# VisionDepth/VisionDepth3D

Measured on AMD Instinct MI355X. Metric: stereo-pairs/sec end-to-end (depth+warp+fill+mux), higher is better.
Workload: dtype f32; 1 GPU; 4k-dav2b-dibr; frame=3840x2160, format=Half-SBS, depth_model=depth-anything-v2-base, depth_net_dtype=float32 (the reference's precision), pixel_overlap=True, pixel_streams=2, clip_frames_all_ranks=32, params=render_cli.py defaults + dof_strength 2.0, dense DOF order (parity mode)

## Files before the change

visiondepth3d_amd/csrc/vd3d_attn.hip:

```cpp
#include "vd3d_dev.h"
#include "vd3d_kernels.h"

#include <mutex>

typedef short at_bf8 __attribute__((ext_vector_type(8)));
typedef float at_f16 __attribute__((ext_vector_type(16)));
typedef uint32_t at_u4 __attribute__((ext_vector_type(4)));

#define AT_D 64
#define AT_BQ 256
#define AT_BK 64
#define AT_NT 512
#define AT_NTERM(MODE) ((MODE) == 0 ? 3 : 2)
#define AT_TILE(MODE) (4 * AT_NTERM(MODE) * 2 * 64 * 16)
#define AT_STAGE(MODE) (2 * AT_TILE(MODE))
#define AT_NSTAGE 3
#define AT_LDS(MODE) (AT_NSTAGE * AT_STAGE(MODE))
#define AT_QBLK(MODE) (4 * AT_NTERM(MODE) * 2 * 32)
#define AT_QKV_SCALE 16.0f
#define AT_P_SCALE 1024.0f
#define AT_OP 272

struct vd_at_args {
  int B, H, T;
// ... 130 lines not shown
    uint8_t* dst = at_lds + buf * STAGE + op * TILE + pp * (AT_NT * 16) + wave_base;
    __builtin_amdgcn_global_load_lds((at_glb_vp)src, (at_lds_vp)dst, 16, 0, 0);
  };

  at_f16 oacc[2];
#pragma unroll
  for (int dm = 0; dm < 2; ++dm)
#pragma unroll
    for (int r = 0; r < 16; ++r) oacc[dm][r] = 0.f;
  float m_run = -INFINITY, l_half = 0.f;

  const int last_tile = a.nkv - 1;
  auto tile_c = [&](int t) { return t < last_tile ? t : last_tile; };
#pragma unroll
  for (int p = 0; p < 6; ++p) dma(0, 0, p);
#pragma unroll
  for (int p = 0; p < 3; ++p) dma(tile_c(1), 1, p);
#pragma unroll
  for (int p = 3; p < 6; ++p) dma(tile_c(1), 1, p);
#pragma unroll
  for (int p = 0; p < 3; ++p) dma(tile_c(2), 2, p);
  if (NP == 3) asm volatile("s_waitcnt vmcnt(6)" ::: "memory"); else asm volatile("s_waitcnt vmcnt(4)" ::: "memory");
  __builtin_amdgcn_s_barrier();

  const int frag_off = (kh * 64 + li) * 16;
  auto st_step = [&](const uint8_t* sk, int ks, at_f16 (&sa)[2]) {
    at_bf8 kf[2][NTERM];
#pragma unroll
    for (int m = 0; m < 2; ++m)
#pragma unroll
      for (int t = 0; t < NTERM; ++t) kf[m][t] = *reinterpret_cast<const at_bf8*>(sk + frag_off + ((ks * NTERM + t) * 2) * 1024 + m * 512);
    AT_MM6(sa[0], kf[0], sa[1], kf[1], qf[ks])
  };
#define AT_CHUNK_HINT(n)                                           \
  __builtin_amdgcn_sched_group_barrier(0x100, 6, 0);               \
  _Pragma("unroll") for (int i_ = 0; i_ < 12; ++i_) {              \
    __builtin_amdgcn_sched_group_barrier(0x008, 1, 0);             \
    __builtin_amdgcn_sched_group_barrier(0x002, n, 0);             \
  }                                                                \
  __builtin_amdgcn_sched_barrier(0);

  at_f16 sacc[2];
#pragma unroll
  for (int m = 0; m < 2; ++m)
#pragma unroll
    for (int r = 0; r < 16; ++r) sacc[m][r] = 0.f;
#pragma unroll
  for (int ks = 0; ks < 4; ++ks) st_step(at_lds, ks, sacc);
  asm volatile("s_waitcnt lgkmcnt(0)" ::: "memory");
  __builtin_amdgcn_s_barrier();

  int cur = 0;
  for (int it = 0; it < a.nkv; ++it) {
    const int s1 = cur == 2 ? 0 : cur + 1, s2 = cur >= 1 ? cur - 1 : 2;
    const uint8_t* sk1 = at_lds + s1 * STAGE;
    const uint8_t* sv = at_lds + cur * STAGE + TILE;
    float z[2][16];
#pragma unroll
    for (int m = 0; m < 2; ++m)
#pragma unroll
      for (int r = 0; r < 16; ++r) z[m][r] = sacc[m][r] * a.c;
    if ((it + 1) * AT_BK > a.T) {
#pragma unroll
      for (int m = 0; m < 2; ++m)
#pragma unroll
        for (int r = 0; r < 16; ++r)
          if (it * AT_BK + 32 * m + (r & 3) + 8 * (r >> 2) + 4 * kh >= a.T) z[m][r] = -INFINITY;
    }
    at_f16 sn[2];
#pragma unroll
    for (int m = 0; m < 2; ++m)
#pragma unroll
      for (int r = 0; r < 16; ++r) sn[m][r] = 0.f;
    dma(tile_c(it + 3), cur, 0);
    __builtin_amdgcn_sched_barrier(0);
    st_step(sk1, 0, sn);
    float mx = -INFINITY;
#pragma unroll
    for (int m = 0; m < 2; ++m)
#pragma unroll
      for (int r = 0; r < 16; ++r) mx = fmaxf(mx, z[m][r]);
    mx = fmaxf(mx, __shfl_xor(mx, 32, 64));
    const float m_new = fmaxf(m_run, mx);
    const float alpha = __builtin_amdgcn_exp2f(m_run - m_new);
    m_run = m_new;
    AT_CHUNK_HINT(2)
    float ps = 0.f;
#pragma unroll
    for (int m = 0; m < 2; ++m) {
      dma(tile_c(it + 3), cur, 1 + m);
      __builtin_amdgcn_sched_barrier(0);
      st_step(sk1, 1 + m, sn);
#pragma unroll
      for (int r = 0; r < 16; ++r) { z[m][r] = __builtin_amdgcn_exp2f(z[m][r] - m_new); ps += z[m][r]; }
      AT_CHUNK_HINT(4)
    }
    dma(tile_c(it + 2), s2, 3);
    __builtin_amdgcn_sched_barrier(0);
    st_step(sk1, 3, sn);
    l_half = l_half * alpha + ps;
#pragma unroll
    for (int dm = 0; dm < 2; ++dm)
#pragma unroll
      for (int r = 0; r < 16; ++r) oacc[dm][r] *= alpha;
    at_bf8 pf[2][NTERM];
    at_split8_m<MODE>(&z[0][0], AT_P_SCALE, pf[0]);
    AT_CHUNK_HINT(7)
#pragma unroll
    for (int ks = 0; ks < 4; ++ks) {
      if (ks < 2) { dma(tile_c(it + 2), s2, 4 + ks); __builtin_amdgcn_sched_barrier(0); }
      if (ks < 3) at_split8_m<MODE>(&z[(ks + 1) >> 1][8 * ((ks + 1) & 1)], AT_P_SCALE, pf[(ks + 1) & 1]);
      at_bf8 vf[2][NTERM];
#pragma unroll
      for (int dm = 0; dm < 2; ++dm)
#pragma unroll
        for (int t = 0; t < NTERM; ++t) vf[dm][t] = *reinterpret_cast<const at_bf8*>(sv + frag_off + ((ks * NTERM + t) * 2) * 1024 + dm * 512);
      AT_MM6(oacc[0], vf[0], oacc[1], vf[1], pf[ks & 1])
      AT_CHUNK_HINT(4)
    }
    if (NP == 3) asm volatile("s_waitcnt vmcnt(6) lgkmcnt(0)" ::: "memory"); else asm volatile("s_waitcnt vmcnt(4) lgkmcnt(0)" ::: "memory");
    __builtin_amdgcn_s_barrier();
#pragma unroll
    for (int m = 0; m < 2; ++m) sacc[m] = sn[m];
    cur = s1;
  }
#undef AT_CHUNK_HINT
  asm volatile("s_waitcnt vmcnt(0)" ::: "memory");
  __builtin_amdgcn_s_barrier();

  const float l_tot = l_half + __shfl_xor(l_half, 32, 64);
  const float inv = MODE == 1 ? 1.0f / (l_tot * (AT_P_SCALE * AT_QKV_SCALE)) : 1.0f / l_tot;
  uint8_t* ow = at_lds + wave * (32 * AT_OP);
#pragma unroll
  for (int dm = 0; dm < 2; ++dm)
#pragma unroll
    for (int g = 0; g < 4; ++g) {
      const float4 v4 = {oacc[dm][4 * g] * inv, oacc[dm][4 * g + 1] * inv, oacc[dm][4 * g + 2] * inv, oacc[dm][4 * g + 3] * inv};
      *reinterpret_cast<float4*>(ow + li * AT_OP + (32 * dm + 8 * g + 4 * kh) * 4) = v4;
    }
  asm volatile("s_waitcnt lgkmcnt(0)" ::: "memory");
  const int b = bh / a.H, h = bh - b * a.H;
#pragma unroll
  for (int i = 0; i < 8; ++i) {
    const int row = i * 4 + (lane >> 4), c4 = lane & 15;
    const int q = q0 + row;
    const float4 v4 = *reinterpret_cast<const float4*>(ow + row * AT_OP + c4 * 16);
    if (q < a.T) *reinterpret_cast<float4*>(out + (((size_t)b * a.T + q) * a.H + h) * AT_D + c4 * 4) = v4;
  }
}

#define AF_TILE (AT_BK * AT_D * 4)
#define AF_STAGE (2 * AF_TILE)
#define AF_LDS (AT_NSTAGE * AF_STAGE)
VD_DEV void af_st(const uint8_t* __restrict__ sk, const float (&qf)[32], int li, int kh, at_f16 (&s)[2]) {
  const int kswz = (li & 15) << 4;
#pragma unroll
  for (int m = 0; m < 2; ++m)
#pragma unroll
    for (int r = 0; r < 16; ++r) s[m][r] = 0.f;
#pragma unroll
  for (int g = 0; g < 8; ++g) {
    float4 kf[2];
#pragma unroll
    for (int m = 0; m < 2; ++m) kf[m] = *reinterpret_cast<const float4*>(sk + (32 * m + li) * 256 + (((8 * kh + g) << 4) ^ kswz));
#pragma unroll
    for (int m = 0; m < 2; ++m) s[m] = __builtin_amdgcn_mfma_f32_32x32x2f32(kf[m].x, qf[4 * g], s[m], 0, 0, 0);
#pragma unroll
    for (int m = 0; m < 2; ++m) s[m] = __builtin_amdgcn_mfma_f32_32x32x2f32(kf[m].y, qf[4 * g + 1], s[m], 0, 0, 0);
#pragma unroll
    for (int m = 0; m < 2; ++m) s[m] = __builtin_amdgcn_mfma_f32_32x32x2f32(kf[m].z, qf[4 * g + 2], s[m], 0, 0, 0);
#pragma unroll
    for (int m = 0; m < 2; ++m) s[m] = __builtin_amdgcn_mfma_f32_32x32x2f32(kf[m].w, qf[4 * g + 3], s[m], 0, 0, 0);
  }
}
VD_DEV void af_pv(const uint8_t* __restrict__ sv, const at_f16 (&p)[2], int li, int kh, at_f16 (&oacc)[2]) {
#pragma unroll
  for (int m = 0; m < 2; ++m)
#pragma unroll
    for (int r = 0; r < 16; ++r) {
      const float2 vv = *reinterpret_cast<const float2*>(sv + (32 * m + (r & 3) + 8 * (r >> 2) + 4 * kh) * 256 + li * 8);
      oacc[0] = __builtin_amdgcn_mfma_f32_32x32x2f32(vv.x, p[m][r], oacc[0], 0, 0, 0);
      oacc[1] = __builtin_amdgcn_mfma_f32_32x32x2f32(vv.y, p[m][r], oacc[1], 0, 0, 0);
    }
}

__global__ __launch_bounds__(AT_NT) void k_attn_f32(const float* __restrict__ qkv, float* __restrict__ out, vd_at_args a) {
  extern __shared__ __attribute__((aligned(16))) uint8_t at_lds[];
  int bh, qb;
  {
    const int wg = blockIdx.x, x = wg & 7, idx = wg >> 3;
    const int g = idx / a.nqb;
    qb = idx - g * a.nqb;
    bh = g * 8 + x;
    if (bh >= a.B * a.H) return;
  }
  const int tid = threadIdx.x, lane = tid & 63, wave = __builtin_amdgcn_readfirstlane(tid >> 6);
  const int li = lane & 31, kh = lane >> 5;
  const int q0 = qb * AT_BQ + wave * 32;
  const int b = bh / a.H, h = bh - b * a.H;
  const size_t tok_stride = (size_t)3 * a.H * AT_D;
  const float* base = qkv + (size_t)b * a.T * tok_stride + h * AT_D;

  const int drow = tid >> 4, dpos = tid & 15, kchunk = dpos ^ (drow & 15);
  auto dma = [&](int tile, int stage) {
    uint8_t* dst = at_lds + stage * AF_STAGE + wave * 1024;
#pragma unroll
    for (int p = 0; p < 2; ++p) {
      const int tok = min(tile * AT_BK + drow + 32 * p, a.T - 1);
      const float* src = base + (size_t)tok * tok_stride + a.H * AT_D;
      __builtin_amdgcn_global_load_lds((at_glb_vp)(src + kchunk * 4), (at_lds_vp)(dst + p * 8192), 16, 0, 0);
      __builtin_amdgcn_global_load_lds((at_glb_vp)(src + a.H * AT_D + dpos * 4), (at_lds_vp)(dst + AF_TILE + p * 8192), 16, 0, 0);
    }
  };

  float qf[32];
  {
    const float4* qp = reinterpret_cast<const float4*>(base + (size_t)min(q0 + li, a.T - 1) * tok_stride + 32 * kh);
#pragma unroll
    for (int g = 0; g < 8; ++g) {
      const float4 v = qp[g];
      qf[4 * g] = v.x * a.c; qf[4 * g + 1] = v.y * a.c; qf[4 * g + 2] = v.z * a.c; qf[4 * g + 3] = v.w * a.c;
    }
  }
  dma(0, 0);
  if (a.nkv > 1) {
    dma(1, 1);
    asm volatile("s_waitcnt vmcnt(4)" ::: "memory");
  } else {
    asm volatile("s_waitcnt vmcnt(0)" ::: "memory");
  }
  __builtin_amdgcn_s_barrier();

  at_f16 oacc[2];
#pragma unroll
  for (int dm = 0; dm < 2; ++dm)
#pragma unroll
    for (int r = 0; r < 16; ++r) oacc[dm][r] = 0.f;
  float m_run = -INFINITY, l_half = 0.f;
  int cur = 0;
  for (int it = 0; it < a.nkv; ++it) {
    const bool ahead = it + 2 < a.nkv;
    if (ahead) dma(it + 2, cur == 0 ? 2 : cur - 1);
    const uint8_t* sk = at_lds + cur * AF_STAGE;
    const uint8_t* sv = sk + AF_TILE;
    at_f16 s[2];
    af_st(sk, qf, li, kh, s);
    if ((it + 1) * AT_BK > a.T) {
#pragma unroll
      for (int m = 0; m < 2; ++m)
#pragma unroll
        for (int r = 0; r < 16; ++r)
          if (it * AT_BK + 32 * m + (r & 3) + 8 * (r >> 2) + 4 * kh >= a.T) s[m][r] = -INFINITY;
    }
    float mx = s[0][0];
#pragma unroll
    for (int m = 0; m < 2; ++m)
#pragma unroll
      for (int r = 0; r < 16; ++r) mx = fmaxf(mx, s[m][r]);
    mx = fmaxf(mx, __shfl_xor(mx, 32, 64));
    const float m_new = fmaxf(m_run, mx);
    if (__any(m_new > m_run)) {
      const float alpha = __builtin_amdgcn_exp2f(m_run - m_new);
#pragma unroll
      for (int dm = 0; dm < 2; ++dm)
#pragma unroll
        for (int r = 0; r < 16; ++r) oacc[dm][r] *= alpha;
      l_half *= alpha;
      m_run = m_new;
    }
    float ps = 0.f;
#pragma unroll
    for (int m = 0; m < 2; ++m)
#pragma unroll
      for (int r = 0; r < 16; ++r) { s[m][r] = __builtin_amdgcn_exp2f(s[m][r] - m_run); ps += s[m][r]; }
    l_half += ps;
    af_pv(sv, s, li, kh, oacc);
    if (ahead) asm volatile("s_waitcnt vmcnt(4) lgkmcnt(0)" ::: "memory"); else asm volatile("s_waitcnt vmcnt(0) lgkmcnt(0)" ::: "memory");
    __builtin_amdgcn_s_barrier();
    cur = cur == 2 ? 0 : cur + 1;
  }

  const float l_tot = l_half + __shfl_xor(l_half, 32, 64);
  const int q = q0 + li;
  if (q < a.T) {
    float* op = out + (((size_t)b * a.T + q) * a.H + h) * AT_D + 8 * kh;
#pragma unroll
    for (int g = 0; g < 4; ++g) {
      const float4 lo = {oacc[0][4 * g] / l_tot, oacc[1][4 * g] / l_tot, oacc[0][4 * g + 1] / l_tot, oacc[1][4 * g + 1] / l_tot};
      const float4 hi = {oacc[0][4 * g + 2] / l_tot, oacc[1][4 * g + 2] / l_tot, oacc[0][4 * g + 3] / l_tot, oacc[1][4 * g + 3] / l_tot};
      *reinterpret_cast<float4*>(op + 16 * g) = lo;
      *reinterpret_cast<float4*>(op + 16 * g + 4) = hi;
    }
  }
}

static bool at_lds_optin(const void* fn, int lds, bool (&done)[64]) {
  static std::mutex mu;
  int dev = 0;
  if (hipGetDevice(&dev) != hipSuccess || dev < 0 || dev >= 64) return false;
  std::lock_guard<std::mutex> lock(mu);
  if (!done[dev]) {
    if (hipFuncSetAttribute(fn, hipFuncAttributeMaxDynamicSharedMemorySize, lds) != hipSuccess) return false;
    done[dev] = true;
  }
  return true;
}

bool vd_launch_attn_f32(hipStream_t s, const float* qkv, int B, int T, int H, int D, float scale, float* out) {
  if (B < 1 || T < 1 || H < 1 || D != AT_D || (long long)B * H > 65535) return false;
  if ((reinterpret_cast<uintptr_t>(qkv) & 15) || (reinterpret_cast<uintptr_t>(out) & 15)) return false;
  static bool attr_set[64] = {};
  if (!at_lds_optin(reinterpret_cast<const void*>(k_attn_f32), AF_LDS, attr_set)) return false;
  vd_at_args a;
  a.B = B; a.H = H; a.T = T;
  a.nq32 = (T + 31) / 32; a.nkv = (T + AT_BK - 1) / AT_BK; a.nqb = (T + AT_BQ - 1) / AT_BQ;
  a.c = scale * 1.44269504088896340736f;
  const int groups = (B * H + 7) / 8;
  hipLaunchKernelGGL(k_attn_f32, dim3((unsigned)(8 * groups * a.nqb)), dim3(AT_NT), AF_LDS, s, qkv, out, a);
  return true;
}

static bool at_mode_ok(int mode) { return mode == 0 || mode == 1; }
long long vd_attn_x3_workspace_bytes(int B, int T, int H, int D, int mode) {
  if (B < 1 || T < 1 || H < 1 || D != AT_D || !at_mode_ok(mode)) return -1;
  const long long nq32 = (T + 31) / 32, nkv = (T + AT_BK - 1) / AT_BK;
  const long long qblk = mode == 0 ? AT_QBLK(0) : AT_QBLK(1), tile = mode == 0 ? AT_TILE(0) : AT_TILE(1);
  return (long long)B * H * (nq32 * qblk * 16 + 2 * nkv * tile);
}

template <int MODE>
static bool at_launch(hipStream_t s, const float* qkv, int B, int T, int H, float scale, void* ws, float* out) {
  static bool attr_set[64] = {};
  if (!at_lds_optin(reinterpret_cast<const void*>(k_attn_bf16x3<MODE>), AT_LDS(MODE), attr_set)) return false;
  vd_at_args a;
  a.B = B; a.H = H; a.T = T;
  a.nq32 = (T + 31) / 32; a.nkv = (T + AT_BK - 1) / AT_BK; a.nqb = (T + AT_BQ - 1) / AT_BQ;
  a.c = scale * 1.44269504088896340736f;
  if (MODE == 1) a.c *= 1.0f / (AT_QKV_SCALE * AT_QKV_SCALE);
  uint4* Qimg = reinterpret_cast<uint4*>(ws);
  uint4* Kimg = Qimg + (size_t)B * H * a.nq32 * AT_QBLK(MODE);
  uint4* Vimg = Kimg + (size_t)B * H * a.nkv * (AT_TILE(MODE) / 16);
  const int rows_max = a.nkv * 64 > a.nq32 * 32 ? a.nkv * 64 : a.nq32 * 32;
  hipLaunchKernelGGL(k_attn_x3_prep<MODE>, dim3((unsigned)((rows_max * 8 + 255) / 256), (unsigned)(B * H), 3), dim3(256), 0, s, qkv, a, Qimg, Kimg, Vimg);
  const int groups = (B * H + 7) / 8;
  hipLaunchKernelGGL(k_attn_bf16x3<MODE>, dim3((unsigned)(8 * groups * a.nqb)), dim3(AT_NT), AT_LDS(MODE), s, Qimg, Kimg, Vimg, out, a);
  return true;
}

bool vd_launch_attn_x3(hipStream_t s, const float* qkv, int B, int T, int H, int D, float scale, void* ws, float* out, int mode) {
  if (vd_attn_x3_workspace_bytes(B, T, H, D, mode) < 0) return false;
  if ((reinterpret_cast<uintptr_t>(qkv) & 15) || (reinterpret_cast<uintptr_t>(ws) & 15) || (reinterpret_cast<uintptr_t>(out) & 15)) return false;
  if ((long long)B * H > 65535) return false;
  return mode == 0 ? at_launch<0>(s, qkv, B, T, H, scale, ws, out) : at_launch<1>(s, qkv, B, T, H, scale, ws, out);
}
```

visiondepth3d_amd/csrc/vd3d_depthprep.hip:

```cpp
#include "vd3d_dev.h"
#include "vd3d_kernels.h"

#define DP_TX 32
#define DP_TY 8
#define DP_KMAX 24

struct vd_prep_args {
  int B, H, W, th, tw;
  float scale_h, scale_w;
  float mean[3], stdv[3];
  int in_rows_max, in_cols_max;
};

VD_DEV float dp_cubic(float x) {
  const float a = -0.5f;
  x = fabsf(x);
  if (x < 1.f) return ((a + 2.f) * x - (a + 3.f)) * x * x + 1.f;
  if (x < 2.f) return (((x - 5.f) * x + 8.f) * x - 4.f) * a;
  return 0.f;
}
VD_DEV int dp_weights(int i, int in, float scale, float* w, int* first) {
  const float support = scale >= 1.f ? 2.f * scale : 2.f;
  const float invscale = scale >= 1.f ? 1.f / scale : 1.f;
  const float center = scale * ((float)i + 0.5f);
  int xmin = (int)(center - support + 0.5f); xmin = xmin < 0 ? 0 : xmin;
  int xend = (int)(center + support + 0.5f); xend = xend > in ? in : xend;
  int n = xend - xmin; n = n > DP_KMAX ? DP_KMAX : n;
  float total = 0.f;
  for (int j = 0; j < n; ++j) { const float v = dp_cubic(((float)(j + xmin) - center + 0.5f) * invscale); w[j] = v; total += v; }
  for (int j = 0; j < n; ++j) w[j] = total != 0.f ? w[j] / total : w[j];
  *first = xmin;
  return n;
}
VD_DEV uint16_t dp_bf16(float f) {
  const uint32_t b = __float_as_uint(f);
  return (uint16_t)((b + 0x7fffu + ((b >> 16) & 1u)) >> 16);
}

VD_DEV void dp_store(uint16_t* o, float f) { *o = dp_bf16(f); }
VD_DEV void dp_store(float* o, float f) { *o = f; }

template <typename OT>
__global__ __launch_bounds__(256) void k_depth_prep(const uint8_t* __restrict__ frames, vd_prep_args a, OT* __restrict__ out) {
  extern __shared__ unsigned char smem[];
  float* wx = reinterpret_cast<float*>(smem);
  float* wy = wx + DP_TX * DP_KMAX;
  int* x0s = reinterpret_cast<int*>(wy + DP_TY * DP_KMAX);
  int* y0s = x0s + 2 * DP_TX;
  float* hb = reinterpret_cast<float*>(y0s + 2 * DP_TY);
  uint8_t* tile = reinterpret_cast<uint8_t*>(hb + (size_t)a.in_rows_max * DP_TX * 3);
  const int tid = threadIdx.x;
  const int ox0 = blockIdx.x * DP_TX, oy0 = blockIdx.y * DP_TY, b = blockIdx.z;
  if (tid < DP_TX) {
    int f = 0, n = 0;
    if (ox0 + tid < a.tw) n = dp_weights(ox0 + tid, a.W, a.scale_w, wx + tid * DP_KMAX, &f);
    x0s[tid] = f; x0s[DP_TX + tid] = n;
  } else if (tid >= 64 && tid < 64 + DP_TY) {
    const int t = tid - 64;
    int f = 0, n = 0;
    if (oy0 + t < a.th) n = dp_weights(oy0 + t, a.H, a.scale_h, wy + t * DP_KMAX, &f);
    y0s[t] = f; y0s[DP_TY + t] = n;
  }
  __syncthreads();
  const int nx = min(DP_TX, a.tw - ox0), ny = min(DP_TY, a.th - oy0);
  const int c_lo = x0s[0], c_hi = x0s[nx - 1] + x0s[DP_TX + nx - 1];
  const int r_lo = y0s[0], r_hi = y0s[ny - 1] + y0s[DP_TY + ny - 1];
  const int ncol = min(c_hi - c_lo, a.in_cols_max), nrow = min(r_hi - r_lo, a.in_rows_max);
  const uint8_t* src = frames + (size_t)b * a.H * a.W * 3;
  const int rowbytes = ncol * 3;
  for (int t = tid; t < nrow * rowbytes; t += 256) {
    const int r = t / rowbytes, cb = t - r * rowbytes;
    tile[(size_t)r * a.in_cols_max * 3 + cb] = src[((size_t)(r_lo + r) * a.W + c_lo) * 3 + cb];
  }
  __syncthreads();
  for (int t = tid; t < nrow * DP_TX; t += 256) {
    const int r = t / DP_TX, ox = t - r * DP_TX;
    float s0 = 0.f, s1 = 0.f, s2 = 0.f;
    if (ox < nx) {
      const int n = x0s[DP_TX + ox];
      const uint8_t* p = tile + (size_t)r * a.in_cols_max * 3 + (size_t)(x0s[ox] - c_lo) * 3;
      const float* w = wx + ox * DP_KMAX;
      for (int j = 0; j < n; ++j) {
        const float wj = w[j];
        s0 += (float)p[3 * j + 2] * wj; s1 += (float)p[3 * j + 1] * wj; s2 += (float)p[3 * j] * wj;
      }
    }
    float* h = hb + ((size_t)r * DP_TX + ox) * 3;
    h[0] = s0; h[1] = s1; h[2] = s2;
  }
  __syncthreads();
  const int ox = tid & (DP_TX - 1), oy = tid / DP_TX;
  if (ox < nx && oy < ny) {
    const int n = y0s[DP_TY + oy], rb = y0s[oy] - r_lo;
    const float* w = wy + oy * DP_KMAX;
    float s[3] = {0.f, 0.f, 0.f};
    for (int j = 0; j < n; ++j) {
      const float* h = hb + ((size_t)(rb + j) * DP_TX + ox) * 3;
      const float wj = w[j];
      s[0] += h[0] * wj; s[1] += h[1] * wj; s[2] += h[2] * wj;
    }
    OT* o = out + (((size_t)b * a.th + (oy0 + oy)) * a.tw + (ox0 + ox)) * 3;
#pragma unroll
    for (int c = 0; c < 3; ++c) dp_store(o + c, ((s[c] / 255.0f) - a.mean[c]) / a.stdv[c]);
  }
}

bool vd_launch_depth_prep(hipStream_t s, const uint8_t* frames, int B, int H, int W, int th, int tw, const float mean[3],
                          const float stdv[3], int dtype, void* out_nhwc) {
  if (dtype != VD3D_DT_BF16 && dtype != VD3D_DT_F32) return false;
  vd_prep_args a;
  a.B = B; a.H = H; a.W = W; a.th = th; a.tw = tw;
  a.scale_h = (float)H / (float)th; a.scale_w = (float)W / (float)tw;
  const float sup_w = a.scale_w >= 1.f ? 2.f * a.scale_w : 2.f, sup_h = a.scale_h >= 1.f ? 2.f * a.scale_h : 2.f;
  if ((int)(2.f * sup_w) + 2 > DP_KMAX || (int)(2.f * sup_h) + 2 > DP_KMAX) return false;
  for (int c = 0; c < 3; ++c) { a.mean[c] = mean[c]; a.stdv[c] = stdv[c]; }
  a.in_cols_max = (int)(a.scale_w * DP_TX + 2.f * sup_w) + 4;
  a.in_rows_max = (int)(a.scale_h * DP_TY + 2.f * sup_h) + 4;
  size_t lds = sizeof(float) * (DP_TX + DP_TY) * DP_KMAX + sizeof(int) * 2 * (DP_TX + DP_TY) +
               sizeof(float) * (size_t)a.in_rows_max * DP_TX * 3 + (size_t)a.in_rows_max * a.in_cols_max * 3;
  lds = (lds + 15) & ~(size_t)15;
  if (lds > 150 * 1024) return false;
  static bool attr[64] = {false};
  int dev = 0;
  (void)hipGetDevice(&dev);
  if (dev >= 0 && dev < 64 && !attr[dev]) {
    (void)hipFuncSetAttribute((const void*)k_depth_prep<uint16_t>, hipFuncAttributeMaxDynamicSharedMemorySize, 160 * 1024);
    (void)hipFuncSetAttribute((const void*)k_depth_prep<float>, hipFuncAttributeMaxDynamicSharedMemorySize, 160 * 1024);
    attr[dev] = true;
  }
  dim3 g((tw + DP_TX - 1) / DP_TX, (th + DP_TY - 1) / DP_TY, B);
  if (dtype == VD3D_DT_F32) hipLaunchKernelGGL(k_depth_prep<float>, g, dim3(256), lds, s, frames, a, reinterpret_cast<float*>(out_nhwc));
  else hipLaunchKernelGGL(k_depth_prep<uint16_t>, g, dim3(256), lds, s, frames, a, reinterpret_cast<uint16_t*>(out_nhwc));
  return true;
}
```

visiondepth3d_amd/csrc/vd3d_handoff.hip:

```cpp
#include "vd3d_dev.h"
#include "vd3d_kernels.h"

struct vd_handoff_args { int B, ph, pw, H, W, invert, same; float sh, sw; };

VD_DEV float cubic1(float x, float A) { return ((A + 2.f) * x - (A + 3.f)) * x * x + 1.f; }
VD_DEV float cubic2(float x, float A) { return ((A * x - 5.f * A) * x + 8.f * A) * x - 4.f * A; }
VD_DEV void cubic_coeffs(float t, float c[4]) {
  const float A = -0.75f;
  c[0] = cubic2(t + 1.f, A); c[1] = cubic1(t, A); c[2] = cubic1(1.f - t, A); c[3] = cubic2((1.f - t) + 1.f, A);
}
VD_DEV float bicubic_at(const float* __restrict__ p, const vd_handoff_args& a, const float cy[4], int iy, int x) {
  const float rx = vd_fma(a.sw, (float)x + 0.5f, -0.5f);
  const float fx = floorf(rx);
  const int ix = (int)fx;
  float cx[4];
  cubic_coeffs(rx - fx, cx);
  int xs[4];
#pragma unroll
  for (int j = 0; j < 4; ++j) { int xx = ix - 1 + j; xs[j] = xx < 0 ? 0 : (xx > a.pw - 1 ? a.pw - 1 : xx); }
  float acc = 0.f;
#pragma unroll
  for (int i = 0; i < 4; ++i) {
    int yy = iy - 1 + i; yy = yy < 0 ? 0 : (yy > a.ph - 1 ? a.ph - 1 : yy);
    const float* row = p + (size_t)yy * a.pw;
    float r = 0.f;
#pragma unroll
    for (int j = 0; j < 4; ++j) r += row[xs[j]] * cx[j];
    acc += r * cy[i];
  }
  return acc;
}
VD_DEV uint32_t f2key(float v) { uint32_t b = __float_as_uint(v); return (b & 0x80000000u) ? ~b : (b | 0x80000000u); }
VD_DEV float key2f(uint32_t k) { uint32_t b = (k & 0x80000000u) ? (k & 0x7fffffffu) : ~k; return __uint_as_float(b); }

__global__ void k_handoff_init(uint32_t* mm, int B) {
  int i = blockIdx.x * blockDim.x + threadIdx.x;
  if (i < B) { mm[3 * i] = 0xffffffffu; mm[3 * i + 1] = 0u; mm[3 * i + 2] = 0u; }
}

#define HO_ROWS 32
template <bool WRITE>
__global__ __launch_bounds__(256) void k_handoff(const float* __restrict__ pred, vd_handoff_args a, uint32_t* __restrict__ mm,
                                                 uint8_t* __restrict__ out) {
  const int b = blockIdx.z;
  const float* p = pred + (size_t)b * a.ph * a.pw;
  const int xq = (blockIdx.x * 64 + (threadIdx.x & 63)) * 4;
  float bmn = INFINITY, bmx = -INFINITY;
  int bbad = 0;
  for (int ry_ = 0; ry_ < HO_ROWS / 4; ++ry_) {
  const int y = blockIdx.y * HO_ROWS + ry_ * 4 + (threadIdx.x >> 6);
  float v[4] = {0.f, 0.f, 0.f, 0.f};
  const bool row_ok = y < a.H;
  if (row_ok && xq < a.W) {
    if (a.same) {
#pragma unroll
      for (int q = 0; q < 4; ++q) if (xq + q < a.W) v[q] = p[(size_t)y * a.W + xq + q];
    } else {
      const float ry = vd_fma(a.sh, (float)y + 0.5f, -0.5f);
      const float fy = floorf(ry);
      float cy[4];
      cubic_coeffs(ry - fy, cy);
#pragma unroll
      for (int q = 0; q < 4; ++q) if (xq + q < a.W) v[q] = bicubic_at(p, a, cy, (int)fy, xq + q);
    }
  }
  if (!WRITE) {
    float mn = INFINITY, mx = -INFINITY;
    int bad = 0;
    if (row_ok)
#pragma unroll
      for (int q = 0; q < 4; ++q)
        if (xq + q < a.W) { bad |= (v[q] != v[q]); mn = v[q] < mn ? v[q] : mn; mx = v[q] > mx ? v[q] : mx; }
    bmn = fminf(bmn, mn); bmx = fmaxf(bmx, mx); bbad |= bad;
  } else {
    if (!row_ok || xq >= a.W) continue;
    const float mn = key2f(mm[3 * b]), mx = key2f(mm[3 * b + 1]);
    const bool flat = mm[3 * b + 2] != 0u || (mx - mn) < (float)1e-6;
    const float den = (mx - mn) + (float)1e-6;
    uint32_t pack = 0;
#pragma unroll
    for (int q = 0; q < 4; ++q) {
      uint8_t u = 0;
      if (!flat) {
        float n = ((v[q] - mn) / den) * 255.f;
        n = n < 0.f ? 0.f : (n > 255.f ? 255.f : n);
        u = (uint8_t)n;
      }
      if (a.invert) u = (uint8_t)(255 - u);
      pack |= (uint32_t)u << (8 * q);
    }
    uint8_t* o = out + (size_t)b * a.H * a.W + (size_t)y * a.W + xq;
    if (xq + 3 < a.W && (((size_t)b * a.H * a.W + (size_t)y * a.W + xq) & 3) == 0) *reinterpret_cast<uint32_t*>(o) = pack;
    else for (int q = 0; q < 4 && xq + q < a.W; ++q) o[q] = (uint8_t)(pack >> (8 * q));
  }
  }
  if (!WRITE) {
    __shared__ float smn[4], smx[4];
    __shared__ int sbad[4];
    for (int off = 32; off > 0; off >>= 1) {
      bmn = fminf(bmn, __shfl_down(bmn, off, 64));
      bmx = fmaxf(bmx, __shfl_down(bmx, off, 64));
      bbad |= __shfl_down(bbad, off, 64);
    }
    if ((threadIdx.x & 63) == 0) { smn[threadIdx.x >> 6] = bmn; smx[threadIdx.x >> 6] = bmx; sbad[threadIdx.x >> 6] = bbad; }
    __syncthreads();
    if (threadIdx.x == 0) {
      const float mn = fminf(fminf(smn[0], smn[1]), fminf(smn[2], smn[3]));
      const float mx = fmaxf(fmaxf(smx[0], smx[1]), fmaxf(smx[2], smx[3]));
      if (mn <= mx) { atomicMin(&mm[3 * b], f2key(mn)); atomicMax(&mm[3 * b + 1], f2key(mx)); }
      if (sbad[0] | sbad[1] | sbad[2] | sbad[3]) atomicOr(&mm[3 * b + 2], 1u);
    }
  }
}

void vd_launch_depth_handoff(hipStream_t s, const float* pred, int B, int ph, int pw, int H, int W, int invert, uint32_t* mm,
                             uint8_t* out) {
  vd_handoff_args a;
  a.B = B; a.ph = ph; a.pw = pw; a.H = H; a.W = W; a.invert = invert; a.same = (ph == H && pw == W);
  a.sh = (float)ph / (float)H; a.sw = (float)pw / (float)W;
  hipLaunchKernelGGL(k_handoff_init, dim3((B + 63) / 64), dim3(64), 0, s, mm, B);
  dim3 g((W + 255) / 256, (H + HO_ROWS - 1) / HO_ROWS, B);
  hipLaunchKernelGGL(k_handoff<false>, g, dim3(256), 0, s, pred, a, mm, out);
  hipLaunchKernelGGL(k_handoff<true>, g, dim3(256), 0, s, pred, a, mm, out);
}
```

Before: 140.1 stereo-pairs/s.

## Skip dead attention tiles, restage depth preprocess, and reuse handoff bicubic rows

Three kernels change. The f32 attention kernel skips compute for waves whose query block is past T and uses a half-width path for short final KV tiles. The depth-prep resize now loads rows per wave into float strips, computes the horizontal pass in registers with taller tiles, and spreads the vertical pass over channels. The handoff bicubic upsample keeps a sliding window of horizontally filtered rows, so each source row is filtered once per column group, and each workgroup covers four times as many rows. This trades redundant loads and math for more register use and new LDS limits, and the prep launcher can now refuse some configurations.

```diff
diff --git a/visiondepth3d_amd/csrc/vd3d_attn.hip b/visiondepth3d_amd/csrc/vd3d_attn.hip
--- a/visiondepth3d_amd/csrc/vd3d_attn.hip
+++ b/visiondepth3d_amd/csrc/vd3d_attn.hip
@@ -306,36 +306,73 @@
 #define AF_TILE (AT_BK * AT_D * 4)
 #define AF_STAGE (2 * AF_TILE)
 #define AF_LDS (AT_NSTAGE * AF_STAGE)
-VD_DEV void af_st(const uint8_t* __restrict__ sk, const float (&qf)[32], int li, int kh, at_f16 (&s)[2]) {
+template <int NM> VD_DEV void af_st(const uint8_t* __restrict__ sk, const float (&qf)[32], int li, int kh, at_f16 (&s)[2]) {
   const int kswz = (li & 15) << 4;
 #pragma unroll
-  for (int m = 0; m < 2; ++m)
+  for (int m = 0; m < NM; ++m)
 #pragma unroll
     for (int r = 0; r < 16; ++r) s[m][r] = 0.f;
 #pragma unroll
   for (int g = 0; g < 8; ++g) {
-    float4 kf[2];
-#pragma unroll
-    for (int m = 0; m < 2; ++m) kf[m] = *reinterpret_cast<const float4*>(sk + (32 * m + li) * 256 + (((8 * kh + g) << 4) ^ kswz));
-#pragma unroll
-    for (int m = 0; m < 2; ++m) s[m] = __builtin_amdgcn_mfma_f32_32x32x2f32(kf[m].x, qf[4 * g], s[m], 0, 0, 0);
-#pragma unroll
-    for (int m = 0; m < 2; ++m) s[m] = __builtin_amdgcn_mfma_f32_32x32x2f32(kf[m].y, qf[4 * g + 1], s[m], 0, 0, 0);
-#pragma unroll
-    for (int m = 0; m < 2; ++m) s[m] = __builtin_amdgcn_mfma_f32_32x32x2f32(kf[m].z, qf[4 * g + 2], s[m], 0, 0, 0);
-#pragma unroll
-    for (int m = 0; m < 2; ++m) s[m] = __builtin_amdgcn_mfma_f32_32x32x2f32(kf[m].w, qf[4 * g + 3], s[m], 0, 0, 0);
-  }
-}
-VD_DEV void af_pv(const uint8_t* __restrict__ sv, const at_f16 (&p)[2], int li, int kh, at_f16 (&oacc)[2]) {
-#pragma unroll
-  for (int m = 0; m < 2; ++m)
+    float4 kf[NM];
+#pragma unroll
+    for (int m = 0; m < NM; ++m) kf[m] = *reinterpret_cast<const float4*>(sk + (32 * m + li) * 256 + (((8 * kh + g) << 4) ^ kswz));
+#pragma unroll
+    for (int m = 0; m < NM; ++m) s[m] = __builtin_amdgcn_mfma_f32_32x32x2f32(kf[m].x, qf[4 * g], s[m], 0, 0, 0);
+#pragma unroll
+    for (int m = 0; m < NM; ++m) s[m] = __builtin_amdgcn_mfma_f32_32x32x2f32(kf[m].y, qf[4 * g + 1], s[m], 0, 0, 0);
+#pragma unroll
+    for (int m = 0; m < NM; ++m) s[m] = __builtin_amdgcn_mfma_f32_32x32x2f32(kf[m].z, qf[4 * g + 2], s[m], 0, 0, 0);
+#pragma unroll
+    for (int m = 0; m < NM; ++m) s[m] = __builtin_amdgcn_mfma_f32_32x32x2f32(kf[m].w, qf[4 * g + 3], s[m], 0, 0, 0);
+  }
+}
+template <int NM> VD_DEV void af_pv(const uint8_t* __restrict__ sv, const at_f16 (&p)[2], int li, int kh, at_f16 (&oacc)[2]) {
+#pragma unroll
+  for (int m = 0; m < NM; ++m)
 #pragma unroll
     for (int r = 0; r < 16; ++r) {
       const float2 vv = *reinterpret_cast<const float2*>(sv + (32 * m + (r & 3) + 8 * (r >> 2) + 4 * kh) * 256 + li * 8);
       oacc[0] = __builtin_amdgcn_mfma_f32_32x32x2f32(vv.x, p[m][r], oacc[0], 0, 0, 0);
       oacc[1] = __builtin_amdgcn_mfma_f32_32x32x2f32(vv.y, p[m][r], oacc[1], 0, 0, 0);
     }
+}
+
+template <int NM, bool MASK>
+VD_DEV void af_tile(const uint8_t* __restrict__ sk, const uint8_t* __restrict__ sv, const float (&qf)[32], int li, int kh, int it, int T, at_f16 (&oacc)[2],
+                    float& m_run, float& l_half) {
+  at_f16 s[2];
+  af_st<NM>(sk, qf, li, kh, s);
+  if (MASK) {
+#pragma unroll
+    for (int m = 0; m < NM; ++m)
+#pragma unroll
+      for (int r = 0; r < 16; ++r)
+        if (it * AT_BK + 32 * m + (r & 3) + 8 * (r >> 2) + 4 * kh >= T) s[m][r] = -INFINITY;
+  }
+  float mx = s[0][0];
+#pragma unroll
+  for (int m = 0; m < NM; ++m)
+#pragma unroll
+    for (int r = 0; r < 16; ++r) mx = fmaxf(mx, s[m][r]);
+  mx = fmaxf(mx, __shfl_xor(mx, 32, 64));
+  const float m_new = fmaxf(m_run, mx);
+  if (__any(m_new > m_run)) {
+    const float alpha = __builtin_amdgcn_exp2f(m_run - m_new);
+#pragma unroll
+    for (int dm = 0; dm < 2; ++dm)
+#pragma unroll
+      for (int r = 0; r < 16; ++r) oacc[dm][r] *= alpha;
+    l_half *= alpha;
+    m_run = m_new;
+  }
+  float ps = 0.f;
+#pragma unroll
+  for (int m = 0; m < NM; ++m)
+#pragma unroll
+    for (int r = 0; r < 16; ++r) { s[m][r] = __builtin_amdgcn_exp2f(s[m][r] - m_run); ps += s[m][r]; }
+  l_half += ps;
+  af_pv<NM>(sv, s, li, kh, oacc);
 }
 
 __global__ __launch_bounds__(AT_NT) void k_attn_f32(const float* __restrict__ qkv, float* __restrict__ out, vd_at_args a) {
@@ -351,6 +388,7 @@
   const int tid = threadIdx.x, lane = tid & 63, wave = __builtin_amdgcn_readfirstlane(tid >> 6);
   const int li = lane & 31, kh = lane >> 5;
   const int q0 = qb * AT_BQ + wave * 32;
+  const bool live = q0 < a.T;
   const int b = bh / a.H, h = bh - b * a.H;
   const size_t tok_stride = (size_t)3 * a.H * AT_D;
   const float* base = qkv + (size_t)b * a.T * tok_stride + h * AT_D;
@@ -397,38 +435,14 @@
     if (ahead) dma(it + 2, cur == 0 ? 2 : cur - 1);
     const uint8_t* sk = at_lds + cur * AF_STAGE;
     const uint8_t* sv = sk + AF_TILE;
-    at_f16 s[2];
-    af_st(sk, qf, li, kh, s);
-    if ((it + 1) * AT_BK > a.T) {
-#pragma unroll
-      for (int m = 0; m < 2; ++m)
-#pragma unroll
-        for (int r = 0; r < 16; ++r)
-          if (it * AT_BK + 32 * m + (r & 3) + 8 * (r >> 2) + 4 * kh >= a.T) s[m][r] = -INFINITY;
-    }
-    float mx = s[0][0];
-#pragma unroll
-    for (int m = 0; m < 2; ++m)
-#pragma unroll
-      for (int r = 0; r < 16; ++r) mx = fmaxf(mx, s[m][r]);
-    mx = fmaxf(mx, __shfl_xor(mx, 32, 64));
-    const float m_new = fmaxf(m_run, mx);
-    if (__any(m_new > m_run)) {
-      const float alpha = __builtin_amdgcn_exp2f(m_run - m_new);
-#pragma unroll
-      for (int dm = 0; dm < 2; ++dm)
-#pragma unroll
-        for (int r = 0; r < 16; ++r) oacc[dm][r] *= alpha;
-      l_half *= alpha;
-      m_run = m_new;
-    }
-    float ps = 0.f;
-#pragma unroll
-    for (int m = 0; m < 2; ++m)
-#pragma unroll
-      for (int r = 0; r < 16; ++r) { s[m][r] = __builtin_amdgcn_exp2f(s[m][r] - m_run); ps += s[m][r]; }
-    l_half += ps;
-    af_pv(sv, s, li, kh, oacc);
+    if (live) {
+      if ((it + 1) * AT_BK > a.T) {
+        if (a.T - it * AT_BK <= 32) af_tile<1, true>(sk, sv, qf, li, kh, it, a.T, oacc, m_run, l_half);
+        else af_tile<2, true>(sk, sv, qf, li, kh, it, a.T, oacc, m_run, l_half);
+      } else {
+        af_tile<2, false>(sk, sv, qf, li, kh, it, a.T, oacc, m_run, l_half);
+      }
+    }
     if (ahead) asm volatile("s_waitcnt vmcnt(4) lgkmcnt(0)" ::: "memory"); else asm volatile("s_waitcnt vmcnt(0) lgkmcnt(0)" ::: "memory");
     __builtin_amdgcn_s_barrier();
     cur = cur == 2 ? 0 : cur + 1;
diff --git a/visiondepth3d_amd/csrc/vd3d_depthprep.hip b/visiondepth3d_amd/csrc/vd3d_depthprep.hip
--- a/visiondepth3d_amd/csrc/vd3d_depthprep.hip
+++ b/visiondepth3d_amd/csrc/vd3d_depthprep.hip
@@ -2,8 +2,10 @@
 #include "vd3d_kernels.h"
 
 #define DP_TX 32
-#define DP_TY 8
+#define DP_TY 26
 #define DP_KMAX 24
+#define DP_NDW 3
+#define DP_HB (DP_TX * 3)
 
 struct vd_prep_args {
   int B, H, W, th, tw;
@@ -48,8 +50,9 @@
   int* x0s = reinterpret_cast<int*>(wy + DP_TY * DP_KMAX);
   int* y0s = x0s + 2 * DP_TX;
   float* hb = reinterpret_cast<float*>(y0s + 2 * DP_TY);
-  uint8_t* tile = reinterpret_cast<uint8_t*>(hb + (size_t)a.in_rows_max * DP_TX * 3);
-  const int tid = threadIdx.x;
+  const int strip = (a.in_cols_max * 3 + 12) & ~3;
+  float* strips = hb + (size_t)a.in_rows_max * DP_HB;
+  const int tid = threadIdx.x, lane = tid & 63, wave = __builtin_amdgcn_readfirstlane(tid >> 6);
   const int ox0 = blockIdx.x * DP_TX, oy0 = blockIdx.y * DP_TY, b = blockIdx.z;
   if (tid < DP_TX) {
     int f = 0, n = 0;
@@ -68,40 +71,89 @@
   const int ncol = min(c_hi - c_lo, a.in_cols_max), nrow = min(r_hi - r_lo, a.in_rows_max);
   const uint8_t* src = frames + (size_t)b * a.H * a.W * 3;
   const int rowbytes = ncol * 3;
-  for (int t = tid; t < nrow * rowbytes; t += 256) {
-    const int r = t / rowbytes, cb = t - r * rowbytes;
-    tile[(size_t)r * a.in_cols_max * 3 + cb] = src[((size_t)(r_lo + r) * a.W + c_lo) * 3 + cb];
+  {
+    const int ox = lane & (DP_TX - 1), half = lane >> 5;
+    const bool col_ok = ox < nx;
+    const int n = col_ok ? x0s[DP_TX + ox] : 0;
+    const int toff = col_ok ? (x0s[ox] - c_lo) * 3 : 0;
+    float w[DP_KMAX];
+#pragma unroll
+    for (int j = 0; j < DP_KMAX; ++j) w[j] = j < n ? wx[ox * DP_KMAX + j] : 0.f;
+    int nmax = n;
+    for (int off = 32; off > 0; off >>= 1) nmax = max(nmax, __shfl_xor(nmax, off, 64));
+    nmax = __builtin_amdgcn_readfirstlane(nmax);
+    float* my = strips + (size_t)wave * 2 * strip;
+    uint32_t dw[2][DP_NDW];
+    int mis[2], ndw[2];
+    auto fetch = [&](int pr) {
+#pragma unroll
+      for (int h = 0; h < 2; ++h) {
+        const int r = min(2 * pr + h, nrow - 1);
+        const uint8_t* g = src + ((size_t)(r_lo + r) * a.W + c_lo) * 3;
+        mis[h] = (int)(reinterpret_cast<uintptr_t>(g) & 3);
+        const uint32_t* g4 = reinterpret_cast<const uint32_t*>(g - mis[h]);
+        ndw[h] = (mis[h] + rowbytes + 3) >> 2;
+#pragma unroll
+        for (int i = 0; i < DP_NDW; ++i)
+          if (64 * i < ndw[h]) dw[h][i] = g4[min(lane + 64 * i, ndw[h] - 1)];
+      }
+    };
+    const int npair = (nrow + 1) >> 1;
+    if (wave < npair) fetch(wave);
+    for (int pr = wave; pr < npair; pr += 4) {
+#pragma unroll
+      for (int h = 0; h < 2; ++h)
+#pragma unroll
+        for (int i = 0; i < DP_NDW; ++i)
+          if (lane + 64 * i < ndw[h]) {
+            const uint32_t v = dw[h][i];
+            const float4 f = {(float)(v & 0xffu), (float)((v >> 8) & 0xffu), (float)((v >> 16) & 0xffu), (float)(v >> 24)};
+            *reinterpret_cast<float4*>(my + h * strip + 4 * (lane + 64 * i)) = f;
+          }
+      const int mis_h = half ? mis[1] : mis[0];
+      if (pr + 4 < npair) fetch(pr + 4);
+      __builtin_amdgcn_fence(__ATOMIC_RELEASE, "wavefront");
+      __builtin_amdgcn_wave_barrier();
+      __builtin_amdgcn_fence(__ATOMIC_ACQUIRE, "wavefront");
+      const int r = 2 * pr + half;
+      if (col_ok && r < nrow) {
+        const float* p = my + half * strip + toff + mis_h;
+        float s0 = 0.f, s1 = 0.f, s2 = 0.f;
+#pragma unroll
+        for (int jc = 0; jc < DP_KMAX; jc += 6) {
+          if (jc >= nmax) break;
+          float x[18];
+#pragma unroll
+          for (int e = 0; e < 18; ++e) x[e] = p[3 * jc + e];
+#pragma unroll
+          for (int j = 0; j < 6; ++j) {
+            const float wj = w[jc + j];
+            const float t0 = s0 + x[3 * j + 2] * wj, t1 = s1 + x[3 * j + 1] * wj, t2 = s2 + x[3 * j] * wj;
+            const bool on = jc + j < n;
+            s0 = on ? t0 : s0; s1 = on ? t1 : s1; s2 = on ? t2 : s2;
+          }
+        }
+        float* h = hb + (size_t)r * DP_HB + ox * 3;
+        h[0] = s0; h[1] = s1; h[2] = s2;
+      }
+      __builtin_amdgcn_fence(__ATOMIC_RELEASE, "wavefront");
+      __builtin_amdgcn_wave_barrier();
+      __builtin_amdgcn_fence(__ATOMIC_ACQUIRE, "wavefront");
+    }
   }
   __syncthreads();
-  for (int t = tid; t < nrow * DP_TX; t += 256) {
-    const int r = t / DP_TX, ox = t - r * DP_TX;
-    float s0 = 0.f, s1 = 0.f, s2 = 0.f;
-    if (ox < nx) {
-      const int n = x0s[DP_TX + ox];
-      const uint8_t* p = tile + (size_t)r * a.in_cols_max * 3 + (size_t)(x0s[ox] - c_lo) * 3;
-      const float* w = wx + ox * DP_KMAX;
-      for (int j = 0; j < n; ++j) {
-        const float wj = w[j];
-        s0 += (float)p[3 * j + 2] * wj; s1 += (float)p[3 * j + 1] * wj; s2 += (float)p[3 * j] * wj;
-      }
-    }
-    float* h = hb + ((size_t)r * DP_TX + ox) * 3;
-    h[0] = s0; h[1] = s1; h[2] = s2;
-  }
-  __syncthreads();
-  const int ox = tid & (DP_TX - 1), oy = tid / DP_TX;
-  if (ox < nx && oy < ny) {
+  for (int t = tid; t < ny * DP_HB; t += 256) {
+    const int oy = t / DP_HB, e = t - oy * DP_HB;
+    if (e >= nx * 3) continue;
+    const int c = e % 3;
     const int n = y0s[DP_TY + oy], rb = y0s[oy] - r_lo;
     const float* w = wy + oy * DP_KMAX;
-    float s[3] = {0.f, 0.f, 0.f};
-    for (int j = 0; j < n; ++j) {
-      const float* h = hb + ((size_t)(rb + j) * DP_TX + ox) * 3;
-      const float wj = w[j];
-      s[0] += h[0] * wj; s[1] += h[1] * wj; s[2] += h[2] * wj;
-    }
-    OT* o = out + (((size_t)b * a.th + (oy0 + oy)) * a.tw + (ox0 + ox)) * 3;
-#pragma unroll
-    for (int c = 0; c < 3; ++c) dp_store(o + c, ((s[c] / 255.0f) - a.mean[c]) / a.stdv[c]);
+    const float* h = hb + (size_t)rb * DP_HB + e;
+    float s = 0.f;
+    for (int j = 0; j < n; ++j) s += h[(size_t)j * DP_HB] * w[j];
+    OT* o = out + (((size_t)b * a.th + (oy0 + oy)) * a.tw + ox0) * 3 + e;
+    const float mc = c == 0 ? a.mean[0] : (c == 1 ? a.mean[1] : a.mean[2]), sc = c == 0 ? a.stdv[0] : (c == 1 ? a.stdv[1] : a.stdv[2]);
+    dp_store(o, ((s / 255.0f) - mc) / sc);
   }
 }
 
@@ -116,8 +168,10 @@
   for (int c = 0; c < 3; ++c) { a.mean[c] = mean[c]; a.stdv[c] = stdv[c]; }
   a.in_cols_max = (int)(a.scale_w * DP_TX + 2.f * sup_w) + 4;
   a.in_rows_max = (int)(a.scale_h * DP_TY + 2.f * sup_h) + 4;
+  if (a.in_cols_max * 3 + 6 > 64 * 4 * DP_NDW) return false;
   size_t lds = sizeof(float) * (DP_TX + DP_TY) * DP_KMAX + sizeof(int) * 2 * (DP_TX + DP_TY) +
-               sizeof(float) * (size_t)a.in_rows_max * DP_TX * 3 + (size_t)a.in_rows_max * a.in_cols_max * 3;
+               sizeof(float) * (size_t)a.in_rows_max * DP_HB + sizeof(float) * (size_t)4 * 2 * ((a.in_cols_max * 3 + 12) & ~3) +
+               sizeof(float) * DP_KMAX * 3;
   lds = (lds + 15) & ~(size_t)15;
   if (lds > 150 * 1024) return false;
   static bool attr[64] = {false};
diff --git a/visiondepth3d_amd/csrc/vd3d_handoff.hip b/visiondepth3d_amd/csrc/vd3d_handoff.hip
--- a/visiondepth3d_amd/csrc/vd3d_handoff.hip
+++ b/visiondepth3d_amd/csrc/vd3d_handoff.hip
@@ -9,27 +9,6 @@
   const float A = -0.75f;
   c[0] = cubic2(t + 1.f, A); c[1] = cubic1(t, A); c[2] = cubic1(1.f - t, A); c[3] = cubic2((1.f - t) + 1.f, A);
 }
-VD_DEV float bicubic_at(const float* __restrict__ p, const vd_handoff_args& a, const float cy[4], int iy, int x) {
-  const float rx = vd_fma(a.sw, (float)x + 0.5f, -0.5f);
-  const float fx = floorf(rx);
-  const int ix = (int)fx;
-  float cx[4];
-  cubic_coeffs(rx - fx, cx);
-  int xs[4];
-#pragma unroll
-  for (int j = 0; j < 4; ++j) { int xx = ix - 1 + j; xs[j] = xx < 0 ? 0 : (xx > a.pw - 1 ? a.pw - 1 : xx); }
-  float acc = 0.f;
-#pragma unroll
-  for (int i = 0; i < 4; ++i) {
-    int yy = iy - 1 + i; yy = yy < 0 ? 0 : (yy > a.ph - 1 ? a.ph - 1 : yy);
-    const float* row = p + (size_t)yy * a.pw;
-    float r = 0.f;
-#pragma unroll
-    for (int j = 0; j < 4; ++j) r += row[xs[j]] * cx[j];
-    acc += r * cy[i];
-  }
-  return acc;
-}
 VD_DEV uint32_t f2key(float v) { uint32_t b = __float_as_uint(v); return (b & 0x80000000u) ? ~b : (b | 0x80000000u); }
 VD_DEV float key2f(uint32_t k) { uint32_t b = (k & 0x80000000u) ? (k & 0x7fffffffu) : ~k; return __uint_as_float(b); }
 
@@ -39,50 +18,93 @@
 }
 
 #define HO_ROWS 32
+#define HO_WG_ROWS (4 * HO_ROWS)
 template <bool WRITE>
 __global__ __launch_bounds__(256) void k_handoff(const float* __restrict__ pred, vd_handoff_args a, uint32_t* __restrict__ mm,
                                                  uint8_t* __restrict__ out) {
   const int b = blockIdx.z;
   const float* p = pred + (size_t)b * a.ph * a.pw;
   const int xq = (blockIdx.x * 64 + (threadIdx.x & 63)) * 4;
+  const int y0 = blockIdx.y * HO_WG_ROWS + __builtin_amdgcn_readfirstlane(threadIdx.x >> 6) * HO_ROWS;
   float bmn = INFINITY, bmx = -INFINITY;
   int bbad = 0;
-  for (int ry_ = 0; ry_ < HO_ROWS / 4; ++ry_) {
-  const int y = blockIdx.y * HO_ROWS + ry_ * 4 + (threadIdx.x >> 6);
+  float cx[4][4];
+  uint32_t xs[4][4];
+  if (!a.same) {
+#pragma unroll
+    for (int q = 0; q < 4; ++q) {
+      const float rx = vd_fma(a.sw, (float)(xq + q) + 0.5f, -0.5f);
+      const float fx = floorf(rx);
+      const int ix = (int)fx;
+      cubic_coeffs(rx - fx, cx[q]);
+#pragma unroll
+      for (int j = 0; j < 4; ++j) { int xx = ix - 1 + j; xs[q][j] = (uint32_t)(xx < 0 ? 0 : (xx > a.pw - 1 ? a.pw - 1 : xx)); }
+    }
+  }
+  float rr[4][4];
+  int wbase = 0;
+  bool wvalid = false;
+  float nmn = 0.f, nmx = 0.f, den = 1.f;
+  bool flat = false;
+  if (WRITE) {
+    nmn = key2f(mm[3 * b]); nmx = key2f(mm[3 * b + 1]);
+    flat = mm[3 * b + 2] != 0u || (nmx - nmn) < (float)1e-6;
+    den = (nmx - nmn) + (float)1e-6;
+  }
+  if (xq < a.W) {
+#pragma unroll 1
+  for (int k = 0; k < HO_ROWS; ++k) {
+  const int y = y0 + k;
+  if (y >= a.H) break;
   float v[4] = {0.f, 0.f, 0.f, 0.f};
-  const bool row_ok = y < a.H;
-  if (row_ok && xq < a.W) {
-    if (a.same) {
+  if (a.same) {
 #pragma unroll
-      for (int q = 0; q < 4; ++q) if (xq + q < a.W) v[q] = p[(size_t)y * a.W + xq + q];
-    } else {
-      const float ry = vd_fma(a.sh, (float)y + 0.5f, -0.5f);
-      const float fy = floorf(ry);
-      float cy[4];
-      cubic_coeffs(ry - fy, cy);
+    for (int q = 0; q < 4; ++q) if (xq + q < a.W) v[q] = p[(size_t)y * a.W + xq + q];
+  } else {
+    const float ry = vd_fma(a.sh, (float)y + 0.5f, -0.5f);
+    const float fy = floorf(ry);
+    const int iy = (int)fy;
+    float cy[4];
+    cubic_coeffs(ry - fy, cy);
+    if (!wvalid || iy < wbase || iy - wbase > 4) { wbase = iy - 4; wvalid = true; }
+#pragma clang loop vectorize(disable) unroll(disable)
+    while (wbase < iy) {
+      ++wbase;
+      int yy = wbase + 2; yy = yy < 0 ? 0 : (yy > a.ph - 1 ? a.ph - 1 : yy);
+      const float* row = p + (size_t)yy * a.pw;
+      float t[4][4];
 #pragma unroll
-      for (int q = 0; q < 4; ++q) if (xq + q < a.W) v[q] = bicubic_at(p, a, cy, (int)fy, xq + q);
+      for (int q = 0; q < 4; ++q)
+#pragma unroll
+        for (int j = 0; j < 4; ++j) t[q][j] = row[xs[q][j]];
+#pragma unroll
+      for (int q = 0; q < 4; ++q) {
+        rr[0][q] = rr[1][q]; rr[1][q] = rr[2][q]; rr[2][q] = rr[3][q];
+        float r = 0.f;
+#pragma unroll
+        for (int j = 0; j < 4; ++j) r += t[q][j] * cx[q][j];
+        rr[3][q] = r;
+      }
+    }
+#pragma unroll
+    for (int q = 0; q < 4; ++q) {
+      float acc = 0.f;
+#pragma unroll
+      for (int i = 0; i < 4; ++i) acc += rr[i][q] * cy[i];
+      v[q] = acc;
     }
   }
   if (!WRITE) {
-    float mn = INFINITY, mx = -INFINITY;
-    int bad = 0;
-    if (row_ok)
 #pragma unroll
-      for (int q = 0; q < 4; ++q)
-        if (xq + q < a.W) { bad |= (v[q] != v[q]); mn = v[q] < mn ? v[q] : mn; mx = v[q] > mx ? v[q] : mx; }
-    bmn = fminf(bmn, mn); bmx = fmaxf(bmx, mx); bbad |= bad;
+    for (int q = 0; q < 4; ++q)
+      if (xq + q < a.W) { bbad |= (v[q] != v[q]); bmn = v[q] < bmn ? v[q] : bmn; bmx = v[q] > bmx ? v[q] : bmx; }
   } else {
-    if (!row_ok || xq >= a.W) continue;
-    const float mn = key2f(mm[3 * b]), mx = key2f(mm[3 * b + 1]);
-    const bool flat = mm[3 * b + 2] != 0u || (mx - mn) < (float)1e-6;
-    const float den = (mx - mn) + (float)1e-6;
     uint32_t pack = 0;
 #pragma unroll
     for (int q = 0; q < 4; ++q) {
       uint8_t u = 0;
       if (!flat) {
-        float n = ((v[q] - mn) / den) * 255.f;
+        float n = ((v[q] - nmn) / den) * 255.f;
         n = n < 0.f ? 0.f : (n > 255.f ? 255.f : n);
         u = (uint8_t)n;
       }
@@ -92,6 +114,7 @@
     uint8_t* o = out + (size_t)b * a.H * a.W + (size_t)y * a.W + xq;
     if (xq + 3 < a.W && (((size_t)b * a.H * a.W + (size_t)y * a.W + xq) & 3) == 0) *reinterpret_cast<uint32_t*>(o) = pack;
     else for (int q = 0; q < 4 && xq + q < a.W; ++q) o[q] = (uint8_t)(pack >> (8 * q));
+  }
   }
   }
   if (!WRITE) {
@@ -119,7 +142,7 @@
   a.B = B; a.ph = ph; a.pw = pw; a.H = H; a.W = W; a.invert = invert; a.same = (ph == H && pw == W);
   a.sh = (float)ph / (float)H; a.sw = (float)pw / (float)W;
   hipLaunchKernelGGL(k_handoff_init, dim3((B + 63) / 64), dim3(64), 0, s, mm, B);
-  dim3 g((W + 255) / 256, (H + HO_ROWS - 1) / HO_ROWS, B);
+  dim3 g((W + 255) / 256, (H + HO_WG_ROWS - 1) / HO_WG_ROWS, B);
   hipLaunchKernelGGL(k_handoff<false>, g, dim3(256), 0, s, pred, a, mm, out);
   hipLaunchKernelGGL(k_handoff<true>, g, dim3(256), 0, s, pred, a, mm, out);
 }
```

Measured after the change: 141.2 stereo-pairs/s, median of 6. No clear change (+0.8%).
